# h3jia/bayesfast

Measured on AMD Instinct MI355X. Metric: leapfrog steps/sec (all chains), 4096 chains x 64-d quadratic surrogate, higher is better.
Workload: dtype f64

## Files before the change

bayesfast_amd/csrc/bfhip_lone.h:

```cpp

#pragma push_macro("exp")
#pragma push_macro("log")
#pragma push_macro("sqrt")
#pragma push_macro("sincospi")
#undef exp
#undef log
#undef sqrt
#undef sincospi
__device__ inline double ln_opq(double x) { asm("" : "+v"(x)); return x; }
#define LN_EXPV(x) ln_opq(exp(ln_opq(x)))
#define LN_LOGV(x) ln_opq(log(ln_opq(x)))
#define LN_SQRTV(x) ln_opq(sqrt(ln_opq(x)))
#define LN_EXP(x) rfl(LN_EXPV(x))
#define LN_LOG(x) rfl(LN_LOGV(x))
#define LN_SQRT(x) rfl(LN_SQRTV(x))

enum { LN_CONT = 0, LN_NEW = 1, LN_DONE = 2 };
enum { LF_NONE = 0, LF_LEAF = 1, LF_INIT = 2 };
enum { LV_CMD = 0, LV_CLOSE, LV_EO, LV_EVAL, LV_DIR, LV_INIT, LV_N = 8 };

template <int W, int DEC>
struct LoneGeo {
    using PG = PipeGeo<W, DEC>;
    static constexpr int DP = 16 * W, NS = 4 * W, NMAT = PG::NMAT, KS = PG::KS, KPJ = PG::KPJ;
    static constexpr int NW = 1 + W, NJ = NMAT * KS;
    static constexpr int NSLOT = SL_PIPE_N;
    static constexpr int o_XT = 0;
    static constexpr int o_GB = o_XT + NMAT * DP;
    static constexpr int o_LF = o_GB + NMAT * KS * DP;
    static constexpr int o_NI = o_LF + 3 * DP + 4;
    static constexpr int o_VD = o_NI + 4 * DP;
    static constexpr int o_WF = o_VD + 2 + LV_N / 2;
    static constexpr int o_LS = o_WF + 4 * DP + 6;
    static constexpr int o_TB = o_LS + BFHIP_MAX_TREEDEPTH * LS_N;
    static constexpr int n_doubles = o_TB + NSLOT * DP;
};

#ifdef BF_LTRACE
#ifndef BF_LTRACE_IDS
#define BF_LTRACE_IDS 0xffff
#endif
#define LTRACE(role, k) do { if (((BF_LTRACE_IDS >> (k)) & 1) && blockIdx.x == 0 && ltrip < BF_LTRACE && lane == 0) LTRC[(ltrip * 2 + (role)) * 16 + (k)] = clock64(); } while (0)
#else
#define LTRACE(role, k) do { } while (0)
#endif

template <int W, int DEC, int NT>
struct LoneJobs {
    using LG = LoneGeo<W, DEC>;
    static constexpr int NJT = LG::NMAT * LG::KS * W, JPW = (NJT + NT - 1) / NT;
    double afr[JPW][LG::KPJ];
    int xoff[JPW], goff[JPW];
    __device__ inline void load(const DevModel &m, int r, int lane) {
#pragma unroll
        for (int u = 0; u < JPW; ++u) {
            const int j = r + u * NT, jj = j < NJT ? j : 0;
            const int mat = jj / (LG::KS * W), rem = jj % (LG::KS * W), kp = rem / W, t = rem % W;
            const double *Af = (mat == 0 ? m.Sf : (mat == 1 ? m.Hf : m.Hdf)) + (t * LG::NS + kp * LG::KPJ) * 64 + lane;
#pragma unroll
            for (int s = 0; s < LG::KPJ; ++s) afr[u][s] = Af[s * 64];
            xoff[u] = (mat * 4 + (lane >> 4)) * LG::NS + kp * LG::KPJ;
            goff[u] = (j < NJT && (lane & 3) == 0) ? (mat * LG::KS + kp) * LG::DP + 16 * t + 4 * ((lane >> 2) & 3) + (lane >> 4) : -1;
        }
    }
    __device__ inline void run(const double *XT, double *GB) const {
        double xb[JPW][LG::KPJ];
#pragma unroll
        for (int u = 0; u < JPW; ++u) {
            const double *xp = XT + xoff[u];
#pragma unroll
            for (int s = 0; s < LG::KPJ; ++s) xb[u][s] = xp[s];
        }
        double acc[JPW];
#pragma unroll
        for (int u = 0; u < JPW; ++u) acc[u] = 0.;
#pragma unroll
        for (int s = 0; s < LG::KPJ; ++s) {
#pragma unroll
            for (int u = 0; u < JPW; ++u) acc[u] = __builtin_amdgcn_mfma_f64_4x4x4f64(afr[u][s], xb[u][s], acc[u], 0, 0, 0);
        }
#pragma unroll
        for (int u = 0; u < JPW; ++u)
            if (goff[u] >= 0) GB[goff[u]] = acc[u];
    }
};

template <int W, int DEC, int FORM = 0> struct LoneWaves {
    static constexpr bool ITILE = true;
    static constexpr int NT = W <= 2 ? 1 : (FORM == 1 ? 3 : W);
    static constexpr int KW = ITILE ? NT : NT + 1;
    static constexpr int NW = KW + 1;
};

template <int W, bool TR, int DEC, int MINW, int FORM = 0>
__global__ __launch_bounds__((LoneWaves<W, DEC, FORM>::NW * 64), MINW) void bf_lone_kernel(DevModel m, SamplerArgs a) {
    using LG = LoneGeo<W, DEC>;
    using LWV = LoneWaves<W, DEC, FORM>;
    constexpr int DP = LG::DP, NS = LG::NS, KS = LG::KS;
    extern __shared__ __attribute__((aligned(16))) double lds[];
    double *XT = lds + LG::o_XT, *GB = lds + LG::o_GB, *LF = lds + LG::o_LF, *NI = lds + LG::o_NI, *VD = lds + LG::o_VD;
    int *VI = (int *)(VD + 2);
    double *LS = lds + LG::o_LS, *TB = lds + LG::o_TB;
#ifdef BF_LTRACE
    __shared__ unsigned long long LTRC[BF_LTRACE * 32];
    for (int i = threadIdx.x; i < BF_LTRACE * 32; i += LWV::NW * 64) LTRC[i] = 0;
    int ltrip = 0;
#endif

    const int tid = threadIdx.x, lane = tid & 63;
    const int w = __builtin_amdgcn_readfirstlane(tid >> 6);
    int chain = blockIdx.x;
    if (a.tail_list) {
        const int cnt = rfl(a.tail_count[0]);
        if ((int)blockIdx.x >= cnt) return;
        chain = rfl(a.tail_list[blockIdx.x]);
    } else if (chain >= a.n_chain) {
        return;
    }
    const int d = m.d;
    const bool lane_ok = lane < DP;

#ifndef LN_ROLE_ONLY
#define LN_ROLE_ONLY -1
#endif
    if (LN_ROLE_ONLY == 0 && w != 0) return;
    if (LN_ROLE_ONLY == 1 && w != LWV::KW) return;
    if (LN_ROLE_ONLY == 2 && (w < 1 || w >= LWV::KW)) return;
    if (w >= 1 && w < LWV::KW) {
        LoneJobs<W, DEC, LWV::NT> jobs;
        jobs.load(m, LWV::ITILE ? w : w - 1, lane);
        for (;;) {
            __syncthreads();
            if (rfl(VI[LV_CMD]) == LN_DONE) break;
            __syncthreads();
            jobs.run(XT, GB);
            __syncthreads();
        }
        return;
    }

    if (w == 0) {
        const double c_lin = lane_ok ? m.pd[PD_LIN * DP + lane] : 0.;
        const double c_mu = lane_ok ? m.pd[PD_MU * DP + lane] : 0.;
        const double c_dmu = (DEC == 1 && lane_ok) ? m.pd[PD_DMU * DP + lane] : 0.;
        const double c_smu = lane_ok ? m.pd[PD_SMU * DP + lane] : 0.;
        const int c_kind = (TR && lane_ok) ? (int)m.pd[PD_KIND * DP + lane] : 0;
        const double c_lo = (TR && lane_ok) ? m.pd[PD_LO * DP + lane] : 0., c_rg = (TR && lane_ok) ? m.pd[PD_RG * DP + lane] : 1.;
        double xs = 0., jac = 1., gj = 0., logdet_l = 0.;
        double q = 0., p = 0., g = 0., var = 1.;
        double eps = 0., eps_t = 0.;
        int dir = 1;
        double *tbl = TB + lane;
        const int xti = (lane & 3) * NS + (lane >> 2);
        LoneJobs<W, DEC, LWV::NT> jobs;
        if constexpr (LWV::ITILE) jobs.load(m, 0, lane);
        for (;;) {
            LTRACE(0, 0);
            __syncthreads();
            LTRACE(0, 1);
            const int4 vw = *(const int4 *)VI;
            const int2 vx = *(const int2 *)(VI + 4);
            const double v_eps_l = VD[0];
            const int cmd = rfl(vw.x), v_close = rfl(vw.y), v_eo = rfl(vw.z), v_eval = rfl(vw.w), v_dir = rfl(vx.x), v_init = rfl(vx.y);
            const double v_eps = rfl(v_eps_l);
            if (cmd == LN_DONE) break;
            bool evaluating = true;
            if (cmd == LN_NEW) {
                q = lane_ok ? NI[lane] : 0.;
                p = lane_ok ? NI[DP + lane] : 0.;
                g = lane_ok ? NI[2 * DP + lane] : 0.;
                var = lane_ok ? NI[3 * DP + lane] : 1.;
                eps = v_eps;
                dir = v_dir;
                eps_t = v_init ? 0. : eps * (double)dir;
            } else {
                int dir_use = dir;
                if (v_close) {
                    const int eo = v_eo;
                    if (lane_ok) { tbl[(eo + 0) * DP] = q; tbl[(eo + 2) * DP] = g; }
                    if (!v_eval) {
                        evaluating = false;
                    } else {
                        dir_use = v_dir;
                        if (dir_use != dir) {
                            const int eo2 = (dir_use > 0) ? SL_RIGHT_Q : SL_LEFT_Q;
                            q = lane_ok ? tbl[(eo2 + 0) * DP] : 0.;
                            p = lane_ok ? tbl[(eo2 + 1) * DP] : 0.;
                            g = lane_ok ? tbl[(eo2 + 2) * DP] : 0.;
                        }
                        dir = dir_use;
                    }
                }
                if (evaluating) eps_t = eps * (double)dir_use;
            }
            if (evaluating) {
                {
                    const double dt = 0.5 * eps_t;
                    p = p + dt * g;
                    q = q + eps_t * (var * p);
                }
                xs = q;
                if constexpr (TR) {
                    double J, J2;
                    bf_to_original(q, c_kind, c_lo, c_rg, xs, J, J2);
                    logdet_l = 0. + LN_LOGV(fabs(J));
                    jac = J;
                    gj = J2 / J;
                }
                if (lane_ok) {
                    XT[xti] = xs;
                    XT[DP + xti] = xs - c_mu;
                    if constexpr (DEC == 1) XT[2 * DP + xti] = xs - c_dmu;
                }
            }
            LTRACE(0, 2);
            __syncthreads();
            LTRACE(0, 3);
            if constexpr (LWV::ITILE) jobs.run(XT, GB);
            LTRACE(0, 7);
            __syncthreads();
            LTRACE(0, 4);
            if (evaluating) {
                auto gb_read = [&](int slot_m) -> double {
                    const double *gp = GB + (slot_m * KS) * DP + lane;
                    double r = gp[0];
                    if (KS > 1) r += gp[DP];
                    return r;
                };
                const double sx = lane_ok ? gb_read(0) : 0.;
                const double hv = lane_ok ? gb_read(1) : 0.;
                const double dgr = DEC == 2 ? hv : ((DEC == 1 && lane_ok) ? gb_read(2) : 0.);
                double gn = sx + c_lin;
                const double xm = xs - c_mu;
                constexpr bool fast_kin = !DEC;
                const double sv = sx - c_smu, gmu = c_smu + c_lin;
                double r_kin = 0., r_val, r_b2, r_bd2 = 0., r_a[2] = {0., 0.};
                if constexpr (DEC == 1) {
                    double r5[5] = {(xs - c_dmu) * dgr, __builtin_fma(0.5 * xs, sx, c_lin * xs), xm * hv, xm * gmu, xm * sv};
                    wave_sum_n<5>(r5);
                    r_bd2 = r5[0]; r_val = r5[1]; r_b2 = r5[2]; r_a[0] = r5[3]; r_a[1] = r5[4];
                } else if constexpr (DEC == 2) {
                    double r4[4] = {__builtin_fma(0.5 * xs, sx, c_lin * xs), xm * hv, xm * gmu, xm * sv};
                    wave_sum_n<4>(r4);
                    r_val = r4[0]; r_b2 = r4[1]; r_a[0] = r4[2]; r_a[1] = r4[3];
                    r_bd2 = r_b2;
                } else {
                    double r3[3] = {0., __builtin_fma(0.5 * xs, sx, c_lin * xs), xm * hv};
                    {
                        double ge = gn * jac;
                        if constexpr (TR) ge += gj;
                        const double pe = p + (0.5 * eps_t) * ge;
                        r3[0] = pe * (var * pe);
                    }
                    wave_sum_n<3>(r3);
                    r_kin = r3[0]; r_val = r3[1]; r_b2 = r3[2];
                }
                LTRACE(0, 5);
                double logdet = 0.;
                if constexpr (TR) logdet = wave_sum(logdet_l);
                double f = (m.c0 + r_val) + 0.;
                double beta = 0.;
                const double a2 = m.alpha * m.alpha;
                if (!(r_b2 < a2 * (1. - 1e-12))) beta = LN_SQRT(r_b2);
                bool kin_ready = fast_kin;
                if (beta > m.alpha) {
                    if constexpr (!DEC) {
                        r_a[0] = xm * gmu; r_a[1] = xm * sv;
                        wave_sum_n<2>(r_a);
                    }
                    const BfOob o = bf_oob_scalars(m.alpha, m.inv_alpha, m.f_mu, m.f_poly_mu, beta, r_a[0], r_a[1]);
                    f = o.f;
                    gn = bf_oob_grad(o, gmu, sv, hv);
                    kin_ready = false;
                }
                gn = gn * jac;
                if constexpr (DEC) {
                    f -= m.decay_gamma * bf_clip0(r_bd2 - m.decay_alpha2);
                    if (r_bd2 > m.decay_alpha2) gn -= 2. * m.decay_gamma * dgr;
                }
                if constexpr (TR) {
                    f += logdet;
                    gn += gj;
                }
                const double logp_new = f;
                const double dt = 0.5 * eps_t;
                p = p + dt * gn;
                g = gn;
                double kin = p * (var * p);
                kin = kin_ready ? r_kin : wave_sum(kin);
                const double E_new = 0.5 * kin - logp_new;
                if (lane_ok) { LF[lane] = q; LF[DP + lane] = p; LF[2 * DP + lane] = g; }
                if (lane == 0) { LF[3 * DP] = E_new; LF[3 * DP + 1] = logp_new; }
            }
            LTRACE(0, 6);
#ifdef BF_LTRACE
            ltrip += 1;
#endif
        }
        return;
    }

    double *scp = a.sc + (size_t)chain * BFHIP_SC_N;
    double *vecp = a.vec + (size_t)chain * BFHIP_VEC_N * d;
    double *tbl = TB + lane;
    const int nw = a.cfg.n_warmup;
    auto load_vec = [&](int field, double pad) -> double { return (lane < d) ? vecp[field * d + lane] : pad; };
    auto store_vec = [&](int field, double v) { if (lane < d) vecp[field * d + lane] = v; };
    auto ldv = [&](int slot) -> double { return lane_ok ? tbl[slot * DP] : 0.; };
    auto stv = [&](int slot, double v) { if (lane_ok) tbl[slot * DP] = v; };
    auto lfv = [&](int k) -> double { return lane_ok ? LF[k * DP + lane] : 0.; };
    double q = 0., p = 0., g = 0., var = 1.;
    double TLp = 0., TPs = 0., TPq = 0., TRp = 0., L0p = 0., L0q = 0., TPg = 0., L0g = 0.;
    uint64_t rs[4], rs_save[4] = {0, 0, 0, 0};
    int i_iter, err;
    double eps = 0.;
    int dir = 1, depth = 0, i_leaf = 0, n_prop = 0, diverged = 0;
    double start_energy = 0., acc_sum = 0., T_W = 0., T_acc = 0., max_de = 0., w_off = 0., L0_W = 0., L0_acc = 0.;
    double E_pend = 0., lp_pend = 0.;
    double log_step, log_bar, hbar, smu, count, step_now, step_bar;
    double prop_E = 0., prop_logp = 0., tree_W = 0., T_E = 0., T_logp = 0.;
    unsigned long long nlf = 0;
    int prev = LF_NONE, fly = LF_NONE;
    bool kdone = false;
    int kb = 0;
    double ad_sq = 0., ad_mk = 0., ad_wgt = 0.;
    bool ad_ready = false;
    double inv_sd = 0.;
    double *WF = lds + LG::o_WF;
#define KBAR() do { if (kb < 2) { __syncthreads(); ++kb; } } while (0)

    auto draw_momentum = [&]() {
        const uint64_t K = bf_xoshiro_next(rs);
        const uint64_t P = (uint64_t)(lane >> 1);
        const double u1 = bf_u01_open0(bf_mix64(K + (2 * P + 1) * BF_GOLDEN));
        const double u2 = bf_u01(bf_mix64(K + (2 * P + 2) * BF_GOLDEN));
        const double rad = LN_SQRTV(-2. * LN_LOGV(u1));
        double sn, cs;
        sincospi(ln_opq(2. * u2), &sn, &cs);
        sn = ln_opq(sn); cs = ln_opq(cs);
        const double z = (lane & 1) ? rad * sn : rad * cs;
        p = (lane < d) ? inv_sd * z : 0.;
        g = 0.;
    };
    auto adapt_consts = [&]() {
        if (!ad_ready && i_iter < nw && a.cfg.adapt_step_size) {
            ad_wgt = 1. / (count + a.cfg.t_0);
            ad_sq = LN_SQRT(count);
            ad_mk = LN_EXP(-a.cfg.k * LN_LOG(count));
            ad_ready = true;
        }
    };
    auto post_new = [&](int init) {
        if (lane_ok) { NI[lane] = q; NI[DP + lane] = p; NI[2 * DP + lane] = g; NI[3 * DP + lane] = var; }
        if (lane == 0) {
            VD[0] = eps;
            VI[LV_CMD] = LN_NEW; VI[LV_CLOSE] = 0; VI[LV_EO] = 0; VI[LV_EVAL] = 1; VI[LV_DIR] = dir; VI[LV_INIT] = init;
        }
    };
    auto init_tree = [&](double E0, double logp0) -> bool {
        if (!(fabs(E0) <= 1.7976931348623157e308)) {
            err = 1;
            for (int k = 0; k < 4; ++k) rs[k] = rs_save[k];
            return false;
        }
        start_energy = E0;
        stv(SL_LEFT_Q, q); stv(SL_LEFT_P, p); stv(SL_LEFT_G, g);
        stv(SL_RIGHT_Q, q); stv(SL_RIGHT_P, p); stv(SL_RIGHT_G, g);
        stv(SL_PROP_Q, q); stv(SL_PSUM, p);
        stv(SL_PROPG, g);
        prop_E = E0;
        prop_logp = logp0;
        tree_W = 1.;
        w_off = 0.;
        max_de = 0.;
        depth = 0; acc_sum = 0.; n_prop = 0; diverged = 0; i_leaf = 0;
        return true;
    };
    auto draw_dir = [&]() {
        for (int k = 0; k < 4; ++k) rs_save[k] = rs[k];
        dir = (bf_u01(bf_xoshiro_next(rs)) < 0.5) ? 1 : -1;
    };

    for (int k = 0; k < 4; ++k) rs[k] = rfl((uint64_t)a.rng[(size_t)chain * 4 + k]);
    log_step = rfl(scp[BFHIP_SC_LOG_STEP]);
    log_bar = rfl(scp[BFHIP_SC_LOG_BAR]);
    hbar = rfl(scp[BFHIP_SC_HBAR]);
    smu = rfl(scp[BFHIP_SC_MU]);
    count = rfl(scp[BFHIP_SC_COUNT]);
    step_now = LN_EXP(log_step);
    step_bar = LN_EXP(log_bar);
    i_iter = rfl((int)scp[BFHIP_SC_I_ITER]);
    err = rfl((int)scp[BFHIP_SC_ERROR]);
    q = load_vec(BFHIP_VEC_Q, 0.);
    var = load_vec(BFHIP_VEC_VAR, 1.);
    inv_sd = 1. / LN_SQRTV(var);
    const bool wf_on = i_iter < nw && a.cfg.adapt_metric;
    if (wf_on) {
        if (lane_ok) {
            WF[lane] = load_vec(BFHIP_VEC_FG_MEAN, 0.); WF[DP + lane] = load_vec(BFHIP_VEC_FG_RAW, 0.);
            WF[2 * DP + lane] = load_vec(BFHIP_VEC_BG_MEAN, 0.); WF[3 * DP + lane] = load_vec(BFHIP_VEC_BG_RAW, 0.);
        }
        if (lane < 5) WF[4 * DP + lane] = scp[BFHIP_SC_FG_N + lane];
    }
    if (i_iter < a.iter_end && err == 0) {
        draw_momentum();
        eps = (i_iter < nw) ? step_now : step_bar;
        draw_dir();
        post_new(1);
        fly = LF_INIT;
    } else {
        if (lane == 0) VI[LV_CMD] = LN_DONE;
        kdone = true;
    }

    for (;;) {
        LTRACE(1, 0);
        __syncthreads();
        LTRACE(1, 1);
        if (kdone) break;
        kb = 0;
        bool ended = false;
        if (prev == LF_INIT) {
            q = lfv(0); p = lfv(1); g = lfv(2);
            const double E0 = rfl(LF[3 * DP]), logp0 = rfl(LF[3 * DP + 1]);
            KBAR(); KBAR();
            if (!init_tree(E0, logp0)) { kdone = true; }
        } else if (prev == LF_LEAF) {
            {
                const double lq_ = lfv(0), lp_ = lfv(1), lg_ = lfv(2);
                const double le_ = LF[3 * DP], ll_ = LF[3 * DP + 1];
                TPq = lq_; TRp = lp_; TPg = lg_;
                E_pend = rfl(le_);
                lp_pend = rfl(ll_);
            }
            LTRACE(1, 4);
            int unit = U_EVAL, lev = 0;
            nlf += 1;
            n_prop += 1;
            double dE = E_pend - start_energy;
            if (dE != dE) dE = INFINITY;
            if (fabs(dE) > fabs(max_de)) max_de = dE;
            T_E = E_pend;
            T_logp = lp_pend;
            T_acc = 0.;
            if (!(fabs(dE) < a.cfg.max_change)) {
                diverged = 1;
                unit = U_ABORT;
            }
            LTRACE(1, 11);
            KBAR();
            LTRACE(1, 10);
            double aw = -dE - w_off;
            const double e_aw = LN_EXPV(aw);
            const double ps0 = L0p + TRp;
            double r2[2] = {ps0 * (var * L0p), ps0 * (var * TRp)};
            wave_sum_n<2>(r2);
            if (unit == U_EVAL) {
                T_W = rfl(e_aw);
                if (aw > 600.) {
                    const double sc_ = LN_EXP(-aw);
                    tree_W = tree_W * sc_;
                    if (lane == 0)
                        for (int l2 = 0; l2 < depth; ++l2) LS[l2 * LS_N + LS_LS] *= sc_;
                    L0_W *= sc_;
                    w_off = w_off + aw;
                    aw = 0.;
                    T_W = 1.;
                }
                const double pacc = (w_off == 0.) ? T_W : LN_EXP(-dE);
                T_acc = pacc > 1. ? 1. : pacc;
                TLp = TRp;
                TPs = TRp;
                unit = U_MERGE;
            }
            LTRACE(1, 5);
            if (unit == U_MERGE && (i_leaf & 1) && depth > 0) {
                T_acc = L0_acc + T_acc;
                const double Wsum = L0_W + T_W;
                if (Wsum != Wsum) err = 2;
                const double u = bf_u01(bf_xoshiro_next(rs));
                lev = 1;
                if ((r2[0] <= 0.) || (r2[1] <= 0.)) {
// ... 282 lines not shown
```

bayesfast_amd/csrc/bfhip_sampler.hip:

```cpp
#include <type_traits>
#include <cstring>
#include <cstdio>
#include <cstdlib>
#include "bfhip_eval.h"
#include "bfhip_metric.h"
#include "bfhip_pld.h"
#include "bfhip_oob.h"

__device__ __attribute__((noinline)) static double bf_exp_ni(double x) { return exp(x); }
__device__ __attribute__((noinline)) static double bf_log_ni(double x) { return log(x); }
__device__ __attribute__((noinline)) static double bf_sqrt_ni(double x) { return sqrt(x); }
__device__ __attribute__((noinline)) static void bf_sincospi_ni(double x, double *s, double *c) { sincospi(x, s, c); }
#define exp(x) bf_exp_ni(x)
#define log(x) bf_log_ni(x)
#define sqrt(x) bf_sqrt_ni(x)
#define sincospi(x, s, c) bf_sincospi_ni(x, s, c)
#define uexp(x) rfl(bf_exp_ni(x))
#define ulog(x) rfl(bf_log_ni(x))
#define usqrt(x) rfl(bf_sqrt_ni(x))

#include "bfhip_sampler_defs.h"

#include "bfhip_wave.h"

// ... 1526 lines not shown
        TRACE(9);
        const int mode_in = mode;
        if constexpr (CHAIN_UNITS) {
            bool first = true;
            do {
                run_unit(first && unit_in == U_EVAL && have_eval, E_new, logp_new);
                first = false;
            } while (unit != U_EVAL && unit != U_DONE);
        } else
        if (unit_in == U_EVAL) run_unit(have_eval, E_new, logp_new);
        else run_unit(false, 0., 0.);
        TRACE(10);
        stamp(unit_in == U_EVAL ? (mode_in == M_INIT ? 4 : 5) : (unit_in == U_MERGE_RUN ? 6 : (unit_in == U_DBL_END ? 7 : (unit_in == U_DONE ? 9 : 8))));
    }

#ifdef BF_TRACE
    if (a.stamps && w == 0 && blockIdx.x == 0)
        for (int i = lane; i < BF_TRACE * 16; i += 64) a.stamps[i] = TRC[i];
#endif
    if constexpr (STAMPS) {
        if (a.stamps && lane == 0)
            for (int k = 0; k < 10; ++k) {
                a.stamps[((size_t)blockIdx.x * 16 + w) * 20 + k] = st_acc[k];
                a.stamps[((size_t)blockIdx.x * 16 + w) * 20 + 10 + k] = st_cnt[k];
            }
    }
    if (real) {
        store_vec(BFHIP_VEC_Q, q);
        if (lane == 0) {
            for (int k = 0; k < 4; ++k) a.rng[(size_t)chain * 4 + k] = rs[k];
            scp[BFHIP_SC_LOG_STEP] = cs_get(CS_LOG_STEP);
            scp[BFHIP_SC_LOG_BAR] = cs_get(CS_LOG_BAR);
            scp[BFHIP_SC_HBAR] = cs_get(CS_HBAR);
            scp[BFHIP_SC_COUNT] = cs_get(CS_COUNT);
            scp[BFHIP_SC_I_ITER] = (double)i_iter;
            scp[BFHIP_SC_ERROR] = (double)err;
            if (a.n_leapfrog && nlf) atomicAdd(a.n_leapfrog, nlf);
        }
    }
}

#ifdef BF_TRACE
#undef TRACE
#define TRACE(k) do { if (w == 0 && blockIdx.x == 0 && trip_no < BF_TRACE && lane == 0) TRC[trip_no * 16 + (k)] = clock64(); } while (0)
#endif
#include "bfhip_nuts_pipe.h"
#include "bfhip_lone.h"

static bool sampler_plain(const DevModel &m) { return bf_model_plain(m) && !bf_tune().no_plain; }

static int sampler_ksplit(const DevModel &m) {
    const int W = m.DP / 16;
    const int n_mat = (m.has_quad ? 1 : 0) + (m.use_bound ? 1 : 0) + (m.use_decay ? 1 : 0);
    int ks = 1;
    while (2 * ks <= W && n_mat * W * 2 * ks <= 16) ks *= 2;
    return ks;
}
static int sampler_gb_slots(const DevModel &m) {
    const int n_mat = (m.has_quad ? 1 : 0) + (m.use_bound ? 1 : 0) + (m.use_decay ? 1 : 0);
    return n_mat * sampler_ksplit(m) > 1 ? n_mat * sampler_ksplit(m) : 1;
}

static size_t sampler_lds_base(const DevModel &m, bool plain) {
    const int W = m.DP / 16, DP = m.DP, NS = 4 * W;
    size_t dbl = (size_t)3 * NS * 65 + (size_t)sampler_gb_slots(m) * 16 * (DP + 1) + (size_t)16 * BFHIP_MAX_TREEDEPTH * LS_N + 4 +
                 (size_t)16 * CS_N + (size_t)PD_N * DP;
    if (DP <= 64 && plain)
        dbl += (size_t)2 * DP * (DP + 2) + (size_t)2 * 16 * DP;
    else if (DP <= 64)
        dbl += (size_t)DP * DP * ((m.has_quad ? 1 : 0) + (m.use_bound ? 1 : 0) + (m.use_decay ? 1 : 0));
    return dbl;
}
static size_t sampler_cubic_doubles(const DevModel &m) {
    return (size_t)2 * m.n2 * m.n2 + (size_t)((m.n3 + 15) >> 4) * m.n3 * m.n3 * 16 + 2;
}
static bool sampler_cubic_lds(const DevModel &m, bool plain) {
    return m.has_cubic && m.n2 <= 64 && m.n3 <= 64 &&
           (sampler_lds_base(m, plain) + sampler_cubic_doubles(m)) * sizeof(double) <= BF_LDS_MAX;
}
static size_t sampler_lds_bytes(const DevModel &m, bool plain, int nwv = 16) {
    if (m.pld.on && m.pld.stream)
        return (((sampler_lds_base(m, false) + 1) & ~(size_t)1) + pld_s_lds_doubles(m.DP, m.pld.MP, m.pld.KC)) * sizeof(double);
    if (m.pld.on)
        return (((sampler_lds_base(m, false) + 1) & ~(size_t)1) +
                pld_lds_doubles(m.DP, m.pld.MP, m.pld.PP, m.pld.KS2, m.pld.n_ent, nwv == 8 ? PLD_XS8 : PLD_XS)) * sizeof(double);
    return (sampler_lds_base(m, plain) + (sampler_cubic_lds(m, plain) ? sampler_cubic_doubles(m) : 0)) * sizeof(double);
}
size_t bf_sampler_lds_bytes_base(const DevModel &m) { return ((sampler_lds_base(m, false) + 1) & ~(size_t)1) * sizeof(double); }

static int wave_layout_cpg(const bfhip_ctx *ctx, int n_chain, int nwv) {
    const int forced = bf_tune().wave_cpg;
    if (forced > 0) return forced < nwv ? forced : nwv;
    int cpg = nwv;
    while (cpg > 1 && (n_chain + cpg / 2 - 1) / (cpg / 2) <= ctx->n_cu) cpg /= 2;
    return cpg;
}

template <int W, bool NUTS, bool STAMPS, int FS, int FULLM = 0>
static int launch_sampler_t(bfhip_ctx *ctx, const SamplerArgs &args_in) {
    BfTune &tune = bf_tune();
    auto k = bf_sampler_kernel<W, NUTS, STAMPS, FS, FULLM>;
    constexpr int NWV = BF_SAMPLER_WAVES(W, FULLM, FS);
    size_t lds = sampler_lds_bytes(ctx->model, FS == 1, NWV);
    SamplerArgs args = args_in;
    args.pld_cl = 0;
    if (ctx->model.pld.on && !ctx->model.pld.stream && NWV == 8 && !tune.pld_no_cl) {
        const size_t with_cl = lds + pld_cl_doubles(ctx->model.pld.MP, ctx->model.pld.PP) * sizeof(double) + 16;
        if (with_cl <= BF_LDS_MAX) { lds = with_cl; args.pld_cl = 1; }
    }
    if (int rc = bf_set_lds(k, lds)) return rc;
    args.cpg = wave_layout_cpg(ctx, args.n_chain, NWV);
    args.cub_lds = sampler_cubic_lds(ctx->model, FS == 1) ? 1 : 0;
    args.cub_loops = tune.cubic_loops;
    const int groups = (args.n_chain + args.cpg - 1) / args.cpg;
    snprintf(tune.last_kernel, sizeof(tune.last_kernel), "bf_sampler_kernel<%d, %s, %s, %d, %d>", W, NUTS ? "true" : "false",
             STAMPS ? "true" : "false", FS, FULLM);
    hipLaunchKernelGGL(k, dim3(groups), dim3(NWV * 64), lds, ctx->stream, ctx->model, args);
    BF_HIP_CHECK(hipGetLastError());
    return 0;
}

extern "C" int bfhip_debug_tail_count(bfhip_ctx *ctx) {
    if (!ctx || !ctx->tail_buf) return -1;
    int n = -1;
    if (hipStreamSynchronize(ctx->stream) != hipSuccess) return -1;
    if (hipMemcpy(&n, ctx->tail_buf, sizeof(int), hipMemcpyDeviceToHost) != hipSuccess) return -1;
    return n;
}
static int tail_stop_now() {
    const BfTune &tune = bf_tune();
    const int hi = tune.lone ? 16 : 4;
    return tune.tail_stop < 1 ? 1 : (tune.tail_stop > hi ? hi : tune.tail_stop);
}

__global__ void bf_tail_list_kernel(int n_chain, int iter_end, const double *sc, int *buf) {
    const int i = blockIdx.x * blockDim.x + threadIdx.x;
    if (i >= n_chain) return;
    const double *scp = sc + (size_t)i * BFHIP_SC_N;
    if ((int)scp[BFHIP_SC_I_ITER] < iter_end && (int)scp[BFHIP_SC_ERROR] == 0) buf[2 + atomicAdd(buf, 1)] = i;
}




template <int W> struct LoneOcc { static constexpr int MINW = W == 1 ? 2 : 3; };

using SamplerKernel = void (*)(DevModel, SamplerArgs);
template <int W, bool TR, int DEC, int FORM>
static SamplerKernel lone_kernel() {
    if constexpr (FORM == 0) return bf_lone_kernel<W, TR, DEC, 1, 0>;
    else if constexpr (FORM == 1) return bf_lone_kernel<W, TR, DEC, 1, (W == 4 ? 1 : 0)>;
    else return bf_lone_kernel<W, TR, DEC, LoneOcc<W>::MINW, 0>;
}
template <int W, int DEC, int FORM> constexpr int lone_threads() { return LoneWaves<W, DEC, (FORM == 1 && W == 4) ? 1 : 0>::NW * 64; }

template <int W, bool TR, int DEC, int FORM>
static int lone_blocks_per_cu(bfhip_ctx *ctx) {
    static int cached[64];
    static bool have[64];
    const int dev = (ctx->device >= 0 && ctx->device < 64) ? ctx->device : 0;
    if (have[dev]) return cached[dev];
    const size_t lds = LoneGeo<W, DEC>::n_doubles * sizeof(double);
    const SamplerKernel k = lone_kernel<W, TR, DEC, FORM>();
    int nb = 0;
    if (bf_set_lds(k, lds) != 0) return 0;
    if (hipOccupancyMaxActiveBlocksPerMultiprocessor(&nb, k, lone_threads<W, DEC, FORM>(), lds) != hipSuccess) return 0;
    cached[dev] = nb;
    have[dev] = true;
    return nb;
}

template <int W, bool TR, int DEC, int FORM>
static int lone_launch_form(bfhip_ctx *ctx, const SamplerArgs &args, int n_blocks) {
    const size_t lds = LoneGeo<W, DEC>::n_doubles * sizeof(double);
    const SamplerKernel k = lone_kernel<W, TR, DEC, FORM>();
    if (int rc = bf_set_lds(k, lds)) return rc;
    hipLaunchKernelGGL(k, dim3(n_blocks), dim3(lone_threads<W, DEC, FORM>()), lds, ctx->stream, ctx->model, args);
    BF_HIP_CHECK(hipGetLastError());
    return 0;
}

template <int W, bool TR, int DEC>
static int launch_lone(bfhip_ctx *ctx, const SamplerArgs &args_in, int n_blocks, bool tail) {
    BfTune &tune = bf_tune();
    if (!tune.lone || args_in.stamps) return 0;
    SamplerArgs args = args_in;
    args.n_cu = ctx->n_cu;
    args.tail_stop = 0;
    args.tail_done = NULL;
    if (!tail) { args.tail_list = NULL; args.tail_count = NULL; }
    args.stamps = tune.stamps_lone;
    const int need = (n_blocks + ctx->n_cu - 1) / ctx->n_cu;
    int form = 0;
    if (lone_blocks_per_cu<W, TR, DEC, 0>(ctx) < need) {
        form = 1;
        if (W != 4 || lone_blocks_per_cu<W, TR, DEC, 1>(ctx) < need) {
            form = 2;
            if (tune.lone != 2 && !tail) return 0;
        }
    }
    if (tune.lone_form >= 0 && tune.lone_form <= 2) form = tune.lone_form;
    const int rc = form == 0 ? lone_launch_form<W, TR, DEC, 0>(ctx, args, n_blocks)
                 : form == 1 ? lone_launch_form<W, TR, DEC, 1>(ctx, args, n_blocks) : lone_launch_form<W, TR, DEC, 2>(ctx, args, n_blocks);
    if (rc) return rc;
    if (!tail) snprintf(tune.last_kernel, sizeof(tune.last_kernel), "bf_lone_kernel<%d, %s, %d, %d>", W, TR ? "true" : "false", DEC, form);
    return 1;
}

template <int W, bool TR = false, int DEC = 0>
static int launch_nuts_pipe(bfhip_ctx *ctx, const SamplerArgs &args_in) {
    BfTune &tune = bf_tune();
    SamplerArgs args = args_in;
    args.cpg = wave_layout_cpg(ctx, args.n_chain, 16);
    args.tail_stop = 0;
    args.tail_list = NULL;
    args.tail_count = NULL;
    args.tail_done = NULL;
    args.n_cu = ctx->n_cu;
    const int quad = tune.no_quad ? 0 : (args.cpg <= 4 ? 1 : (args.cpg <= 8 ? 2 : 0));
    auto k = quad == 1 ? bf_nuts_pipe_kernel<W, TR, DEC, 1> : (quad == 2 ? bf_nuts_pipe_kernel<W, TR, DEC, 2> : bf_nuts_pipe_kernel<W, TR, DEC, 0>);
    if ((quad == 1 && tune.wave_cpg == 0) || tune.lone == 2) {
        const int r = launch_lone<W, TR, DEC>(ctx, args, args.n_chain, false);
        if (r != 0) return r < 0 ? r : 0;
    }
    const size_t lds = PipeGeo<W, DEC>::lds_doubles() * sizeof(double);
    if (int rc = bf_set_lds(k, lds)) return rc;
    const int groups = (args.n_chain + args.cpg - 1) / args.cpg;
    const bool two_parts = tune.tail_relaunch && args.cpg == 16 && !tune.no_quad && !args.stamps;
    if (two_parts) {
        if (int rc = bf_grow(ctx, (void **)&ctx->tail_buf, &ctx->tail_bytes, (size_t)(args.n_chain + 2) * sizeof(int))) return rc;
        args.tail_stop = tail_stop_now();
        args.tail_q = tune.tail_q < 1 ? 1 : (tune.tail_q > 4 ? 4 : tune.tail_q);
        args.tail_done = ctx->tail_buf + 1;
        BF_HIP_CHECK(hipMemsetAsync(ctx->tail_buf, 0, 2 * sizeof(int), ctx->stream));
    }
    hipLaunchKernelGGL(k, dim3(groups), dim3(1024), lds, ctx->stream, ctx->model, args);
    BF_HIP_CHECK(hipGetLastError());
    snprintf(tune.last_kernel, sizeof(tune.last_kernel), "bf_nuts_pipe_kernel<%d, %s, %d, %d>", W, TR ? "true" : "false", DEC, quad);
    if (two_parts) {
        hipLaunchKernelGGL(bf_tail_list_kernel, dim3((args.n_chain + 255) / 256), dim3(256), 0, ctx->stream, args.n_chain, args.iter_end, args.sc,
                           ctx->tail_buf);
        BF_HIP_CHECK(hipGetLastError());
        auto k2 = bf_nuts_pipe_kernel<W, TR, DEC, 1>;
        if (int rc = bf_set_lds(k2, lds)) return rc;
        SamplerArgs a2 = args;
        a2.tail_stop = 0;
        a2.tail_count = ctx->tail_buf;
        a2.tail_list = ctx->tail_buf + 2;
        a2.tail_done = NULL;
        a2.cpg = 4;
        {
            const int most = args.n_chain < args.tail_stop * groups ? args.n_chain : args.tail_stop * groups;
            const int r = launch_lone<W, TR, DEC>(ctx, a2, most, true);
            if (r != 0) return r < 0 ? r : 0;
        }
        const int groups2 = groups > ctx->n_cu ? groups : ctx->n_cu;
        hipLaunchKernelGGL(k2, dim3(groups2), dim3(1024), lds, ctx->stream, ctx->model, a2);
        BF_HIP_CHECK(hipGetLastError());
    }
    return 0;
}

template <int W, bool NUTS>
static int launch_sampler(bfhip_ctx *ctx, const SamplerArgs &args) {
    const BfTune &tune = bf_tune();
    const DevModel &m = ctx->model;
    const bool plain = sampler_plain(m) && !args.mat;
    if (m.pld.on && m.pld.stream) {
        if (sampler_lds_bytes(m, false, 8) > BF_LDS_MAX)
            return bf_set_error(BFHIP_ERR_UNSUPPORTED, "bfhip_sampler_run: this streamed pipeline density needs %zu KB of LDS at d = %d (160 KB)",
                                sampler_lds_bytes(m, false, 8) / 1024, m.d);
        return args.mat ? launch_sampler_t<W, NUTS, false, 11, 1>(ctx, args) : launch_sampler_t<W, NUTS, false, 11>(ctx, args);
    }
    if (m.pld.on) {
        if constexpr (W == 8) {
            if (sampler_lds_bytes(m, false, 8) > BF_LDS_MAX)
                return bf_set_error(BFHIP_ERR_UNSUPPORTED, "bfhip_sampler_run: this pipeline density needs %zu KB of LDS at d = %d (160 KB)",
                                    sampler_lds_bytes(m, false, 8) / 1024, m.d);
            return args.mat ? launch_sampler_t<8, NUTS, false, 9, 1>(ctx, args) : launch_sampler_t<8, NUTS, false, 9>(ctx, args);
        } else {
            if (args.mat) {
                return launch_sampler_t<W, NUTS, false, 9, 1>(ctx, args);
            }
            const long gemm_steps = (long)m.pld.NT1 * m.pld.NS1 + (long)m.pld.NT2 * m.pld.NS2;
            const bool w8 = m.pld.only8 || (tune.pld_waves ? tune.pld_waves == 8 : (args.n_chain <= 8 * ctx->n_cu || gemm_steps <= 800));
            if (w8 && m.has_transform && m.has_su && m.use_bound && !m.use_decay && !tune.no_plain) return launch_sampler_t<W, NUTS, false, 10>(ctx, args);
            return w8 ? launch_sampler_t<W, NUTS, false, 9>(ctx, args) : launch_sampler_t<W, NUTS, false, 8>(ctx, args);
        }
    }
    if (args.mat) {
        const bool adapting = args.cfg.adapt_metric && args.iter_out0 < args.cfg.n_warmup;
        return (adapting || tune.no_vel_ahead) ? launch_sampler_t<W, NUTS, false, 0, 1>(ctx, args) : launch_sampler_t<W, NUTS, false, 0, 2>(ctx, args);
    }
#ifndef BF_TRACE
    if (W == 4 && NUTS && args.stamps)
        return plain ? launch_sampler_t<W, NUTS, (W == 4 && NUTS), (W == 4 && NUTS) ? 1 : 0>(ctx, args)
                     : launch_sampler_t<W, NUTS, (W == 4 && NUTS), 0>(ctx, args);
    const bool stamped = args.stamps != NULL;
#else
    const bool stamped = false;
#endif
    const bool common = bf_common_surrogate(m) && !tune.no_plain;
    const bool pipe = NUTS && !tune.no_pipe && !stamped;
    if constexpr (W <= 4) {
        if (plain && pipe) return launch_nuts_pipe<W>(ctx, args);
    }
    if (plain) return launch_sampler_t<W, NUTS, false, 1>(ctx, args);
    if constexpr (W <= 4) {
        if (pipe && common && m.has_transform && !m.use_decay) return launch_nuts_pipe<W, true>(ctx, args);
        if (pipe && common && m.use_decay && !m.has_transform) {
            if (m.decay_shared && !tune.no_decay_shared) return launch_nuts_pipe<W, false, 2>(ctx, args);
            return launch_nuts_pipe<W, false, 1>(ctx, args);
        }
    }
#ifndef BF_ONLY_HEADLINE
    if constexpr (W == 4) {
        if (common) {
            switch (bf_feature_bits(m)) {
            case 7: return launch_sampler_t<4, NUTS, false, 7>(ctx, args);
            case 3: return launch_sampler_t<4, NUTS, false, 3>(ctx, args);
            case 5: return launch_sampler_t<4, NUTS, false, 5>(ctx, args);
            }
        }
    }
    if constexpr (W == 8 && NUTS) {
        if (!tune.no_plain && m.has_quad && m.use_bound && m.has_cubic && !m.use_decay && !m.has_transform && !m.has_su && !m.has_link) {
            const int form = tune.cubic_form;
// ... 196 lines not shown
```

Measured before the change: 721.1 million.

## Replace post-job workgroup barrier with atomic counter handover in lone kernel

Job waves no longer hit a second __syncthreads after computing their matrix tiles. Each instead bumps a workgroup-scoped atomic counter in LDS, and the leader wave spins on that counter until every job wave has posted. This removes one full block barrier per leapfrog step and lets job waves loop back to the next command barrier early. It also moves the DEC==1 c_dmu constant into LDS when multiple blocks per CU are used, to ease register pressure. The cost is spin-wait overhead and reliance on correct release/acquire fencing.

```diff
diff --git a/bayesfast_amd/csrc/bfhip_lone.h b/bayesfast_amd/csrc/bfhip_lone.h
--- a/bayesfast_amd/csrc/bfhip_lone.h
+++ b/bayesfast_amd/csrc/bfhip_lone.h
@@ -17,7 +17,21 @@
 
 enum { LN_CONT = 0, LN_NEW = 1, LN_DONE = 2 };
 enum { LF_NONE = 0, LF_LEAF = 1, LF_INIT = 2 };
-enum { LV_CMD = 0, LV_CLOSE, LV_EO, LV_EVAL, LV_DIR, LV_INIT, LV_N = 8 };
+enum { LV_CMD = 0, LV_CLOSE, LV_EO, LV_EVAL, LV_DIR, LV_INIT, LV_JOBS, LV_N = 8 };
+
+#ifdef BF_LONE_B2_BARRIER
+#define LN_HANDOVER 0
+#else
+#define LN_HANDOVER 1
+#endif
+__device__ inline void ln_jobs_post(int *cnt, int lane) {
+    __builtin_amdgcn_fence(__ATOMIC_RELEASE, "wavefront");
+    if (lane == 0) __hip_atomic_fetch_add(cnt, 1, __ATOMIC_RELEASE, __HIP_MEMORY_SCOPE_WORKGROUP);
+}
+__device__ inline void ln_jobs_wait(const int *cnt, unsigned target) {
+    while ((int)((unsigned)rfl(__hip_atomic_load(cnt, __ATOMIC_RELAXED, __HIP_MEMORY_SCOPE_WORKGROUP)) - target) < 0) __builtin_amdgcn_s_sleep(1);
+    __builtin_amdgcn_fence(__ATOMIC_ACQUIRE, "workgroup");
+}
 
 template <int W, int DEC>
 struct LoneGeo {
@@ -33,7 +47,8 @@
     static constexpr int o_WF = o_VD + 2 + LV_N / 2;
     static constexpr int o_LS = o_WF + 4 * DP + 6;
     static constexpr int o_TB = o_LS + BFHIP_MAX_TREEDEPTH * LS_N;
-    static constexpr int n_doubles = o_TB + NSLOT * DP;
+    static constexpr int o_CD = o_TB + NSLOT * DP;
+    template <int MINW> static constexpr int n_doubles() { return o_CD + ((DEC == 1 && MINW > 1) ? DP : 0); }
 };
 
 #ifdef BF_LTRACE
@@ -134,7 +149,15 @@
             if (rfl(VI[LV_CMD]) == LN_DONE) break;
             __syncthreads();
             jobs.run(XT, GB);
+#if LN_HANDOVER
+            ln_jobs_post(VI + LV_JOBS, lane);
+#else
             __syncthreads();
+#endif
+#ifdef BF_LTRACE
+            if (w == 1) LTRACE(0, 8);
+            ltrip += 1;
+#endif
         }
         return;
     }
@@ -142,7 +165,11 @@
     if (w == 0) {
         const double c_lin = lane_ok ? m.pd[PD_LIN * DP + lane] : 0.;
         const double c_mu = lane_ok ? m.pd[PD_MU * DP + lane] : 0.;
-        const double c_dmu = (DEC == 1 && lane_ok) ? m.pd[PD_DMU * DP + lane] : 0.;
+        constexpr bool dmu_lds = DEC == 1 && MINW > 1;
+        const double c_dmu = (DEC == 1 && !dmu_lds && lane_ok) ? m.pd[PD_DMU * DP + lane] : 0.;
+        if constexpr (dmu_lds) {
+            if (lane_ok) lds[LG::o_CD + lane] = m.pd[PD_DMU * DP + lane];
+        }
         const double c_smu = lane_ok ? m.pd[PD_SMU * DP + lane] : 0.;
         const int c_kind = (TR && lane_ok) ? (int)m.pd[PD_KIND * DP + lane] : 0;
         const double c_lo = (TR && lane_ok) ? m.pd[PD_LO * DP + lane] : 0., c_rg = (TR && lane_ok) ? m.pd[PD_RG * DP + lane] : 1.;
@@ -154,6 +181,11 @@
         const int xti = (lane & 3) * NS + (lane >> 2);
         LoneJobs<W, DEC, LWV::NT> jobs;
         if constexpr (LWV::ITILE) jobs.load(m, 0, lane);
+#if LN_HANDOVER
+        constexpr int n_post = LWV::KW - 1;
+        unsigned jobs_target = 0;
+        if (n_post > 0 && lane == 0) VI[LV_JOBS] = 0;
+#endif
         for (;;) {
             LTRACE(0, 0);
             __syncthreads();
@@ -210,7 +242,7 @@
                 if (lane_ok) {
                     XT[xti] = xs;
                     XT[DP + xti] = xs - c_mu;
-                    if constexpr (DEC == 1) XT[2 * DP + xti] = xs - c_dmu;
+                    if constexpr (DEC == 1) XT[2 * DP + xti] = xs - (dmu_lds ? lds[LG::o_CD + lane] : c_dmu);
                 }
             }
             LTRACE(0, 2);
@@ -218,7 +250,17 @@
             LTRACE(0, 3);
             if constexpr (LWV::ITILE) jobs.run(XT, GB);
             LTRACE(0, 7);
+#if LN_HANDOVER
+            if constexpr (n_post > 0) {
+                jobs_target += n_post;
+                ln_jobs_wait(VI + LV_JOBS, jobs_target);
+            } else {
+                __builtin_amdgcn_fence(__ATOMIC_RELEASE, "wavefront");
+                __builtin_amdgcn_wave_barrier();
+            }
+#else
             __syncthreads();
+#endif
             LTRACE(0, 4);
             if (evaluating) {
                 auto gb_read = [&](int slot_m) -> double {
@@ -236,7 +278,8 @@
                 const double sv = sx - c_smu, gmu = c_smu + c_lin;
                 double r_kin = 0., r_val, r_b2, r_bd2 = 0., r_a[2] = {0., 0.};
                 if constexpr (DEC == 1) {
-                    double r5[5] = {(xs - c_dmu) * dgr, __builtin_fma(0.5 * xs, sx, c_lin * xs), xm * hv, xm * gmu, xm * sv};
+                    const double c_dmu_c = dmu_lds ? (lane_ok ? lds[LG::o_CD + lane] : 0.) : c_dmu;
+                    double r5[5] = {(xs - c_dmu_c) * dgr, __builtin_fma(0.5 * xs, sx, c_lin * xs), xm * hv, xm * gmu, xm * sv};
                     wave_sum_n<5>(r5);
                     r_bd2 = r5[0]; r_val = r5[1]; r_b2 = r5[2]; r_a[0] = r5[3]; r_a[1] = r5[4];
                 } else if constexpr (DEC == 2) {
@@ -327,7 +370,7 @@
     bool ad_ready = false;
     double inv_sd = 0.;
     double *WF = lds + LG::o_WF;
-#define KBAR() do { if (kb < 2) { __syncthreads(); ++kb; } } while (0)
+#define KBAR() do { if (kb < (LN_HANDOVER ? 1 : 2)) { __syncthreads(); ++kb; } } while (0)
 
     auto draw_momentum = [&]() {
         const uint64_t K = bf_xoshiro_next(rs);
diff --git a/bayesfast_amd/csrc/bfhip_sampler.hip b/bayesfast_amd/csrc/bfhip_sampler.hip
--- a/bayesfast_amd/csrc/bfhip_sampler.hip
+++ b/bayesfast_amd/csrc/bfhip_sampler.hip
@@ -1702,6 +1702,9 @@
     else if constexpr (FORM == 1) return bf_lone_kernel<W, TR, DEC, 1, (W == 4 ? 1 : 0)>;
     else return bf_lone_kernel<W, TR, DEC, LoneOcc<W>::MINW, 0>;
 }
+template <int W, int DEC, int FORM> constexpr size_t lone_lds_bytes() {
+    return LoneGeo<W, DEC>::template n_doubles<FORM == 2 ? LoneOcc<W>::MINW : 1>() * sizeof(double);
+}
 template <int W, int DEC, int FORM> constexpr int lone_threads() { return LoneWaves<W, DEC, (FORM == 1 && W == 4) ? 1 : 0>::NW * 64; }
 
 template <int W, bool TR, int DEC, int FORM>
@@ -1710,7 +1713,7 @@
     static bool have[64];
     const int dev = (ctx->device >= 0 && ctx->device < 64) ? ctx->device : 0;
     if (have[dev]) return cached[dev];
-    const size_t lds = LoneGeo<W, DEC>::n_doubles * sizeof(double);
+    const size_t lds = lone_lds_bytes<W, DEC, FORM>();
     const SamplerKernel k = lone_kernel<W, TR, DEC, FORM>();
     int nb = 0;
     if (bf_set_lds(k, lds) != 0) return 0;
@@ -1722,7 +1725,7 @@
 
 template <int W, bool TR, int DEC, int FORM>
 static int lone_launch_form(bfhip_ctx *ctx, const SamplerArgs &args, int n_blocks) {
-    const size_t lds = LoneGeo<W, DEC>::n_doubles * sizeof(double);
+    const size_t lds = lone_lds_bytes<W, DEC, FORM>();
     const SamplerKernel k = lone_kernel<W, TR, DEC, FORM>();
     if (int rc = bf_set_lds(k, lds)) return rc;
     hipLaunchKernelGGL(k, dim3(n_blocks), dim3(lone_threads<W, DEC, FORM>()), lds, ctx->stream, ctx->model, args);
```

Result: no change. 726.7 million (median of 6 runs) (+0.8%).
